# Sudaraka88/LDWeaver

Measured on AMD Instinct MI355X. Metric: MI SNP-pairs/sec, higher is better.
Workload: dtype i8

## Files before the change

### ldweaver_amd/csrc/ldw_apx.h

```cpp
#pragma once
#include "ldw_internal.h"
#include "ldw_epi.h"

namespace ldw {

constexpr int APX_TW = 128;
struct ApxGemmArgs {
    const uint64_t *panel_t, *panel_f;
    int RTpad, RFpad, M2;
    const uint8_t *dig_a, *dig_b;
    const int32_t *shift;
    int32_t *G;
    int lower_only;
    int fine;
    int fuse;
    const uint8_t *bin_t, *bin_f;
    const int2 *tab;
    int tab_nb;
    uint8_t *clean;
    const uint8_t *sr_mask;
    unsigned long long *skip_ctr;
    uint32_t *tile_list;
    unsigned int *n_live;
    int grid_wgs;
// ... 12 lines not shown
```

### ldweaver_amd/csrc/ldw_apx.hip

```cpp
#include <algorithm>
#include <cmath>
#include <cstdlib>

#include "ldw_apx.h"
#include "ldw_pairs.h"
#include "ldw_dev.h"

using namespace ldw;

namespace ldw {

namespace {
constexpr int64_t APX_PROD_CAP = 12000;
struct ProdTable {
    std::vector<int32_t> val;
    std::vector<uint8_t> a, b;
    ProdTable() {
        std::vector<std::pair<int32_t, std::pair<uint8_t, uint8_t>>> all;
        for (int x = 0; x <= 127; ++x)
            for (int y = x; y <= 127; ++y) all.push_back({x * y, {(uint8_t)x, (uint8_t)y}});
        std::sort(all.begin(), all.end());
        for (auto &e : all)
            if (val.empty() || val.back() != e.first) {
                val.push_back(e.first);
// ... 85 lines not shown
    c->apx.apx_ok = delta <= 4e-3 && Npad <= 30720 && M2 > 0;
    {
        char why[160];
        if (c->apx.apx_ok) snprintf(why, sizeof(why), c->apx.apx_fine ? "ok (block exponents per 32 positions)" : "ok");
        else if (!(delta <= 4e-3)) snprintf(why, sizeof(why), "delta %.3g > 4e-03 (dual-digit weights too coarse)", delta);
        else if (Npad > 30720) snprintf(why, sizeof(why), "Npad %lld > 30720 (digit arrays exceed the GEMM's LDS)", (long long)Npad);
        else snprintf(why, sizeof(why), "no macro step (Npad %lld)", (long long)Npad);
        c->apx.apx_gate = why;
    }
    return LDW_OK;
}

__global__ __launch_bounds__(256) void k_pack_panel(const uint64_t *__restrict__ Mbits, int64_t KW, const int32_t *__restrict__ rowlist,
                                                    int Rpad, int M2, uint64_t *__restrict__ panel, int interleave,
                                                    const int32_t *__restrict__ rowlist2 = nullptr, int Rpad2 = 0, uint64_t *__restrict__ panel2 = nullptr) {
    typedef unsigned long long u64x2 __attribute__((ext_vector_type(2)));
    typedef unsigned int u32x4 __attribute__((ext_vector_type(4)));
    if (blockIdx.y == 1) {
        rowlist = rowlist2;
        Rpad = Rpad2;
        panel = panel2;
    }
    const int r = blockIdx.x * 64 + (threadIdx.x & 63);
    if (r >= Rpad) return;
    const u64x2 *src = reinterpret_cast<const u64x2 *>(Mbits + (int64_t)rowlist[r] * KW);
    u32x4 *dst4 = reinterpret_cast<u32x4 *>(panel);
    for (int m = threadIdx.x >> 6; m < M2; m += 4) {
        u64x2 v = src[m];
        if (interleave) {
            const unsigned long long x = v[0], y = v[1];
            const unsigned long long ex = (x & 0xFFFFull) | ((x >> 16) & 0xFFFF0000ull) | ((y & 0xFFFFull) << 32) | ((y << 16) & 0xFFFF000000000000ull);
            const unsigned long long ox = ((x >> 16) & 0xFFFFull) | ((x >> 32) & 0xFFFF0000ull) | (((y >> 16) & 0xFFFFull) << 32) | (y & 0xFFFF000000000000ull);
            v[0] = ex;
            v[1] = ox;
        }
#pragma unroll
        for (int h = 0; h < 2; ++h) {
            const unsigned long long w = v[h];
            u32x4 o;
#pragma unroll
            for (int kk = 0; kk < 4; ++kk)
                o[kk] = (((unsigned int)(w >> (16 * kk)) & 0xFFu) << 3) | (((unsigned int)(w >> (16 * kk + 8)) & 0xFFu) << 19);
            dst4[((int64_t)m * Rpad + r) * 2 + h] = o;
        }
    }
}

int launch_pack_panel(ldw_ctx *c, const int32_t *rowlist, int Rpad, uint64_t *panel, hipStream_t st, const int32_t *rowlist2, int Rpad2, uint64_t *panel2) {
    const int rmax = (rowlist2 && Rpad2 > Rpad) ? Rpad2 : Rpad;
    hipLaunchKernelGGL(k_pack_panel, dim3((unsigned)((rmax + 63) / 64), rowlist2 ? 2u : 1u), dim3(256), 0, st, c->rows.Mbits.as<uint64_t>(), c->KW, rowlist, Rpad,
                       (int)(c->KW / 2), panel, c->apx.apx_fine ? 1 : 0, rowlist2, Rpad2, panel2);
    LDW_HIP(hipGetLastError());
    return LDW_OK;
}

typedef int v4i __attribute__((ext_vector_type(4)));
typedef int v16i __attribute__((ext_vector_type(16)));
constexpr int APX_MT = 4, APX_WPS = 2;

typedef unsigned int apx_u32x4 __attribute__((ext_vector_type(4)));
// ... 122 lines not shown
            S.bmin = v < S.bmin ? v : S.bmin;
            S.bmax = v > S.bmax ? v : S.bmax;
        }
        if (flags) {
            const uint4 f = *reinterpret_cast<const uint4 *>(flags + i);
            unsigned a = f.x & f.y & f.z & f.w, o = f.x | f.y | f.z | f.w;
            a &= a >> 16; a &= a >> 8;
            o |= o >> 16; o |= o >> 8;
            S.fand &= a & 0xFFu;
            S.forr |= o & 0xFFu;
        }
    }
    return S;
}

__global__ __launch_bounds__(256) void k_apx_live_tiles(ApxGemmArgs P) {
    constexpr int MT = APX_MT, NT = 2, TH = 32 * MT, TWd = 32 * NT;
    __shared__ unsigned int s_wave[4], s_base;
    const int ty = (int)blockIdx.x, ntx = P.RFpad / TWd;
    const int lane = threadIdx.x & 63, wave = threadIdx.x >> 6;
    const TileSummary T = apx_fold_rows(P.bin_t + (int64_t)ty * TH, P.rflag_t ? P.rflag_t + (int64_t)ty * TH : nullptr, TH);
    unsigned int n_pruned = 0;
    for (int tx0 = 0; tx0 < ntx; tx0 += 256) {
        const int tx = tx0 + (int)threadIdx.x;
        const bool valid = tx < ntx && !(P.lower_only && tx * TWd + TWd - 1 < ty * TH);
        bool pruned = false, all_binned = false;
        if (valid && !(P.sr_mask && P.sr_mask[(int64_t)((ty * TH) / 128) * (P.RFpad / 64) + tx] != 0)) {
            const TileSummary F = apx_fold_rows(P.bin_f + (int64_t)tx * TWd, P.rflag_f ? P.rflag_f + (int64_t)tx * TWd : nullptr, TWd);
            all_binned = T.bmax < P.tab_nb && F.bmax < P.tab_nb;
            if (P.rflag_t) {
                const unsigned kt = T.fand & PF_KIND, kf = F.fand & PF_KIND;
                pruned = kt >= 2u && kt == (T.forr & PF_KIND) && kf >= 2u && kf == (F.forr & PF_KIND) &&
                         ((T.fand & (kf == 2u ? PF_DEAD2 : PF_DEAD3)) != 0u || (F.fand & (kt == 2u ? PF_DEAD2 : PF_DEAD3)) != 0u);
            }
            if (!pruned && all_binned && (T.bmax - T.bmin + 1) * (F.bmax - F.bmin + 1) <= 64) {
                bool ok = true;
                for (int bt = T.bmin; bt <= T.bmax; ++bt)
                    for (int bf = F.bmin; bf <= F.bmax; ++bf) {
                        const int2 th = P.tab[bt * P.tab_nb + bf];
                        ok = ok && th.x < 0 && th.y == 2147483647;
                    }
                pruned = ok;
            }
        }
        if (pruned && all_binned) {
#pragma unroll
            for (int i = 0; i < MT; ++i)
#pragma unroll
                for (int h = 0; h < (NT * 32) / 64; ++h) P.clean[(int64_t)((ty * TH + 32 * i) / 32) * (P.RFpad / 64) + (tx * TWd) / 64 + h] = 1;
        }
        const bool live = valid && !pruned;
        const unsigned long long lm = __ballot(live);
        n_pruned += (unsigned int)__popcll(__ballot(valid && pruned));
        if (lane == 0) s_wave[wave] = (unsigned int)__popcll(lm);
        __syncthreads();
        if (threadIdx.x == 0) {
            const unsigned int tot = s_wave[0] + s_wave[1] + s_wave[2] + s_wave[3];
// ... 207 lines not shown
```

### ldweaver_amd/csrc/ldw_mi.hip

```cpp
#include <algorithm>
#include <chrono>
#include <cmath>
#include <cstring>
#include "ldw_prim.h"

#include "ldw_internal.h"
#include "ldw_dev.h"
#ifndef LDW_SCREEN_V
#define LDW_SCREEN_V 2
#endif
#ifndef LDW_SCREEN_WAVES
#define LDW_SCREEN_WAVES 6
#endif
#include "ldw_epi.h"
#include "ldw_pass_plan.h"
#include <future>

#include "ldw_apx.h"
#include "ldw_pairs.h"

using namespace ldw;

namespace ldw {
#include "ldw_mi_screen.inc"
// ... 73 lines not shown
        if (int rc = c->cand_val[s].reserve(cand * 8)) return rc;
        if (int rc = gx(c, s).reserve(RF * RF * 8)) return rc;
    }
    if (int rc = c->pair_sums.reserve((size_t)PAIR_PATHS * PAIR_SHARDS * cap * 16 * 8)) return rc;
    return LDW_OK;
}

int block_mi_dense(ldw_ctx *c, const int32_t *from_idx, int64_t nf, const int32_t *to_idx, int64_t nt, int quirk) {
    EmitArgs E;
    memset(&E, 0, sizeof(E));
    return run_block_mi(c, from_idx, nf, to_idx, nt, quirk, E);
}

void warm_mi() {
    hipFuncAttributes a;
    (void)hipFuncGetAttributes(&a, reinterpret_cast<const void *>(&k_zero4));
    (void)hipFuncGetAttributes(&a, reinterpret_cast<const void *>(&k_mi_screen<1, true>));
    (void)hipGetLastError();
}
}

extern "C" {

int ldw_mi_block(ldw_ctx *c, const int32_t *from_idx, int64_t nf, const int32_t *to_idx, int64_t nt, int quirk_mode,
                 double *MI_out, int on_device) {
    if (int rc = check_gpu(c)) return rc;
    LDW_REQUIRE(from_idx && to_idx && MI_out, LDW_ERR_ARG, "ldw_mi_block: null argument");
    LDW_REQUIRE(quirk_mode == LDW_QUIRK_REFERENCE || quirk_mode == LDW_QUIRK_INTENDED, LDW_ERR_ARG, "bad quirk mode");
    EmitArgs E;
    memset(&E, 0, sizeof(E));
    if (int rc = run_block_mi(c, from_idx, nf, to_idx, nt, quirk_mode, E)) return rc;
// ... 463 lines not shown
```

### ldweaver_amd/csrc/ldw_mi_block.inc

```

int upload_i32(ldw_ctx *c, ldw::DevBuf &buf, const std::vector<int32_t> &v) {
    if (int rc = buf.reserve(v.size() * 4 + 4)) return rc;
    if (!v.empty()) LDW_HIP(hipMemcpyAsync(buf.p, v.data(), v.size() * 4, hipMemcpyHostToDevice, c->stream));
    return LDW_OK;
}

struct SideLists {
    std::vector<int32_t> rowlist, lrow, pos;
    std::vector<uint8_t> cls;
    int Rpad = 0;
};

int build_side(ldw_ctx *c, const int32_t *idx, int64_t n, SideLists &S, const std::vector<int32_t> *order1 = nullptr) {
    S.lrow.assign((size_t)n, 0);
    S.rowlist.clear();
    S.pos.clear();
    S.cls.clear();
    const int32_t zero_row = (int32_t)c->rows.R;
    for (int64_t k = 0; k < n; ++k)
        LDW_REQUIRE(idx[k] >= 0 && idx[k] < c->L, LDW_ERR_ARG, "SNP index %d out of range 0..%lld", idx[k], (long long)c->L - 1);
    for (int cl : {1, 2, 4}) {
        const bool ordered = cl == 1 && order1 != nullptr;
        const int64_t cnt = ordered ? (int64_t)order1->size() : n;
        for (int64_t kk = 0; kk < cnt; ++kk) {
// ... 503 lines not shown
    }
    const bool maybe_on = getenv("LDW_NO_MAYBE") == nullptr;
    const bool use_maybe = maybe_on && !c->spec.maybe_off && fuse && use_pairs && c->knobs.screen == 1 && !E.lower_only && c->KW >= 32;
    unsigned int *maybe_n = nullptr;
    ApxMaybe *maybe_list = nullptr;
    MiniCol *mini_c = nullptr;
    MiniRow *mini_r = nullptr;
    if (use_maybe) {
        maybe_n = PL.hdr + PH_MAYBE_N;
        maybe_list = PL.maybe;
        if (int rc = place(M, c->apx_mini[s])) return rc;
        A.mini_c = mini_c = M.col;
        A.mini_r = mini_r = M.row;
    }
    if (phase == 1) {
        if (E.do_lr) {
            if (int rc = launch_pack_panel(c, D.rl_f, RFpad, c->panel[s][0].as<uint64_t>(), gs, lo_h->diag ? nullptr : D.rl_t, RTpad,
                                           lo_h->diag ? nullptr : c->panel[s][1].as<uint64_t>()))
                return rc;
        }
        {
            ZeroArgs Z;
            memset(&Z, 0, sizeof(Z));
            auto zero = [&Z](int k, const Carve::Range &r) {
                Z.p[k] = reinterpret_cast<uint4 *>(r.p);
                Z.n16[k] = r.n16();
            };
            zero(0, U.zeroed());
            if (use_pairs) zero(1, PL.zeroed());
            if (fuse) {
                Z.p[4] = reinterpret_cast<uint4 *>(c->apx_clean[s].p);
                Z.n16[4] = (unsigned int)(((size_t)(RTpad / 32) * (size_t)(RFpad / 64) + 15) / 16);
            }
            zero(5, B.zeroed());
            if (zero_hist) {
                Z.p[2] = reinterpret_cast<uint4 *>(zero_hist);
                Z.n16[2] = (unsigned int)((size_t)NBINS * 8 / 16 * (size_t)(lo_h->span ? lo_h->span : 1));
                Z.p[3] = reinterpret_cast<uint4 *>(zero_pick);
                Z.n16[3] = (unsigned int)(zero_pick_bytes / 16);
            }
            hipLaunchKernelGGL(k_zero4, dim3(16), dim3(256), 0, gs, Z);
        }
        const int nthr = std::max<int>(std::max<int>((int)nt, (int)g.nf_slots()), std::max<int>(RTpad, RFpad));
        hipLaunchKernelGGL(k_build_packs, dim3((unsigned)((nthr + 255) / 256), 2), dim3(256), 0, gs, A, D.perm, D.perm_t, (int)g.nf_slots(), 1, K.cp, K.cp_hi, K.rp,
                           K.rp_hi, K.rloc_f, K.rloc_t, B.bin_t, B.bin_f, RTpad, RFpad, sflag_f, sflag_t, rflag_f, rflag_t, mini_c, mini_r);
        LDW_HIP(hipGetLastError());
        ApxGemmArgs P;
        if (E.do_lr) {
            memset(&P, 0, sizeof(P));
            P.panel_f = c->panel[s][0].as<uint64_t>();
            P.panel_t = lo_h->diag ? P.panel_f : c->panel[s][1].as<uint64_t>();
            P.RTpad = RTpad;
            P.RFpad = RFpad;
            P.M2 = (int)(c->KW / 2);
            P.dig_a = c->apx.dig_a.as<uint8_t>();
            P.dig_b = c->apx.dig_b.as<uint8_t>();
            P.shift = c->apx.apx_shift.as<int32_t>();
            P.fine = c->apx.apx_fine ? 1 : 0;
            P.G = c->Gapx[s].as<int32_t>();
            P.lower_only = E.lower_only;
// ... 64 lines not shown
    if (need_exact && !band_early)
        if (int rc = launch_gemm_bits(c, c->rows.Mbits.as<uint64_t>(), c->KW, D.rl_t, RTpad, D.rl_f, RFpad, Gx.as<int64_t>(), c->wts.nlimbs, c->wts.digits.as<int8_t>(),
                                      E.lower_only, s2, 0, -1, band, band ? D.band_list : nullptr, D.n_band))
            return rc;
    if (use_pairs) {
        if (int rc = c->pair_sums.reserve((size_t)PAIR_PATHS * PAIR_SHARDS * A.pl_cap * 16 * 8)) return rc;
        if (int rc = launch_pairs_exact(c, A, ghist, c->pair_sums.as<int64_t>(), s2)) return rc;
    }
    if (need_exact) {
        EpiArgs Ax = A;
        Ax.G = Gx.as<int64_t>();
        Ax.E.apx = 0;
        Ax.pl_pairs = nullptr;
        launch_units(Ax, D, U, ghist, s2);
    }
    hipLaunchKernelGGL(k_apx_stats, dim3(1), dim3(64), 0, s2, U.counters, A.pl_n, A.pl_cap, A.E.scr_viol + 1);
    LDW_HIP(hipGetLastError());
    LDW_HIP(hipEventRecord(ev[2], s2));
    return LDW_OK;
}

void build_perm_tiles(ldw_ctx *c, const int32_t *from_idx, int64_t nf, std::vector<int32_t> &perm, const std::vector<int32_t> *order1 = nullptr) {
    perm.clear();
    for (int want : {1, 2, 3, 4, 0}) {
        if (want == 1 && order1) perm.insert(perm.end(), order1->begin(), order1->end());
        else
            for (int64_t k = 0; k < nf; ++k)
                if (c->rows.h_row0[from_idx[k] + 1] - c->rows.h_row0[from_idx[k]] == want) perm.push_back((int32_t)k);
        if (want != 3)
            while (perm.size() % 64) perm.push_back(-1);
    }
    if (perm.empty()) perm.assign(64, -1);
// ... 107 lines not shown
```

### ldweaver_amd/csrc/ldw_mi_eval.inc

```
#ifndef LDW_EPI_WAVES
#define LDW_EPI_WAVES 3
#endif
#ifndef LDW_EPI_FAST_WAVES
#define LDW_EPI_FAST_WAVES 5
#endif
#ifndef LDW_EPI_U11
#define LDW_EPI_U11 4
#endif
#ifndef LDW_EPI_U
#define LDW_EPI_U 2
#endif
struct EpiFastConst {
    double den, rY, hrcp, rxy0;
};
__device__ __forceinline__ bool col_is_fast_r(const ColMeta &M, uint32_t mb) { return col_is_fast(mb) && M.rb == (double)((int)(mb & 7) + 1); }

template <int MODE>
__device__ __forceinline__ void epi_fast_emit(const EmitArgs &E, const ColMeta &M, int a_loc, int b_loc, int sa, double mi, unsigned int *sh_hist) {
    if (E.write_dense) E.MI[(int64_t)a_loc + (int64_t)b_loc * E.nf] = mi;
    if (MODE == 0) return;
    if (a_loc == b_loc) return;
    const int seg = a_loc > b_loc ? 1 : 0;
    if (E.any_sr) {
        const ColInfo &c = M.ci;
// ... 328 lines not shown
                    g_viol_rec[k * 4 + 1] = (double)M.sb;
                    g_viol_rec[k * 4 + 2] = mi;
                    g_viol_rec[k * 4 + 3] = (double)A.E.spec_lo;
                }
            }
            continue;
        }
        emit_pair_spec(A.E, M.ci, a_loc, b_loc, R.sa, M.sb, mi, ghist);
    }
}

struct ZeroArgs {
    uint4 *p[6];
    unsigned int n16[6];
};
__global__ __launch_bounds__(256) void k_zero4(ZeroArgs Z) {
    const uint4 z = make_uint4(0u, 0u, 0u, 0u);
#pragma unroll
    for (int k = 0; k < 6; ++k)
        for (unsigned int i = blockIdx.x * 256u + threadIdx.x; i < Z.n16[k]; i += gridDim.x * 256u) Z.p[k][i] = z;
}

__global__ void k_apx_stats(const unsigned int *__restrict__ n_units, const unsigned int *__restrict__ pl_n, unsigned int pl_cap,
                            unsigned long long *__restrict__ acc) {
    if (threadIdx.x != 0 || blockIdx.x != 0) return;
    acc[0] += (unsigned long long)n_units[0] + n_units[1];
    unsigned long long k = 0;
    if (pl_n)
        for (int i = 0; i < PAIR_PATHS * PAIR_SHARDS; ++i) k += pl_n[i] > pl_cap ? pl_cap : pl_n[i];
    acc[1] += k;
    if (pl_n) acc[2] += (unsigned long long)pl_n[PH_MAYBE_N];
}

struct GenArgs {
    const double *MI;
    int nf, nt, lower_only, keep_sr, do_lr;
    const int32_t *idx_f, *idx_t, *POS;
    double g, sr_dist;
};

__device__ __forceinline__ bool gen_is_sr(const GenArgs &S, int a_loc, double pos1) {
    return circ_len(pos1, (double)S.POS[S.idx_f[a_loc]], S.g) <= S.sr_dist;
}

__global__ __launch_bounds__(256) void k_gen_count(GenArgs S, int32_t *__restrict__ cnt_u, int32_t *__restrict__ cnt_l,
                                                   unsigned long long *__restrict__ ghist) {
// ... 106 lines not shown
```

### ldweaver_amd/csrc/ldw_mi_items.inc

```

struct StageImage {
    struct Part {
        size_t off, bytes;
        const void *src;
        void (*point)(DevPtrs &, const char *);
    };
    Part part[18] = {};
    int n = 0;
    size_t bytes = 0;
    template <class T> static T elem_of(const T *DevPtrs::*);
    template <auto F> using Elem = decltype(elem_of(F));
    template <auto F> size_t array(const Elem<F> *src, size_t count) {
        part[n] = Part{bytes, count * sizeof(Elem<F>), src, [](DevPtrs &D, const char *p) { D.*F = reinterpret_cast<const Elem<F> *>(p); }};
        bytes = (bytes + part[n].bytes + 63) / 64 * 64;
        return part[n++].off;
    }
    void copy_to(char *image) const {
        for (int k = 0; k < n; ++k)
            if (part[k].src && part[k].bytes) memcpy(image + part[k].off, part[k].src, part[k].bytes);
    }
    void bind(DevPtrs &D, const char *image) const {
        for (int k = 0; k < n; ++k) part[k].point(D, image + part[k].off);
    }
};
// ... 425 lines not shown
    E.scr_mode = (hb.spec_B > 0 || !do_lr) && !E.write_dense && (!do_lr || speculation_pays(c, p)) ? c->knobs.screen : 0;
    const int64_t tot = hb.mixed ? c->wts.total_fixed_hi : c->wts.total_fixed;
    int bits = 0;
    while (bits < 62 && (tot >> bits) != 0) ++bits;
    E.scr_shift = bits > 31 ? bits - 31 : 0;
    E.scr_scale = (float)std::ldexp(1.0, E.scr_shift - c->wts.frac_bits + (hb.mixed ? 8 * LO_LIMBS : 0));
    E.scr_eps = SCREEN_EPS + (hb.mixed ? (float)lo_bound(c) : 0.0f);
    if (hb.apx) {
        apx_screen_params(c, E);
    }
    E.scr_viol = reinterpret_cast<unsigned long long *>(sl.lr_count + 1);
    hb.E = E;
    return LDW_OK;
}

int launch_pick(ldw_ctx *c, const HostBlock &hb, const ldw_mi_params *p, const SmallLayout &sl, hipStream_t st) {
    const int s = hb.slot;
    const unsigned int *pl_hdr = c->pairs[s].as<unsigned int>();
    if (hb.span) {
        PickSpanArgs S;
        memset(&S, 0, sizeof(S));
        for (int k = 0; k < hb.span; ++k) S.n_total[k] = (long long)hb.seg_lr_total[k];
        hipLaunchKernelGGL(k_pick_bucket_span, dim3((unsigned)hb.span), dim3(256), 0, st, c->hist[s].as<unsigned long long>(), p->lr_retain_links,
                           p->lr_links_approx, hb.spec_B, S, reinterpret_cast<char *>(sl.pick[s]), PICK_STRIDE,
                           pl_hdr, pair_cap_for(hb.nf, hb.nt, hb.span));
        LDW_HIP(hipGetLastError());
        return LDW_OK;
    }
    if (!p->sr_only) {
        const bool pl = hb.apx && c->knobs.screen == 1;
        hipLaunchKernelGGL(k_pick_bucket, dim3(1), dim3(256), 0, st, c->hist[s].as<unsigned long long>(), p->lr_retain_links,
                           p->lr_links_approx, hb.spec_B, (long long)hb.n_lr_total, sl.pick[s],
                           pl ? pl_hdr : nullptr, pair_cap_for(hb.nf, hb.nt));
        LDW_HIP(hipGetLastError());
    }
    return LDW_OK;
}

static void fill_dev_ptrs(ldw_ctx *c, HostBlock &hb) {
    hb.img.bind(hb.D, c->dstage[hb.pin_slot >= 0 ? hb.pin_slot : hb.slot].as<char>() + hb.stage_base);
}

int submit_upload(ldw_ctx *c, HostBlock &hb) {
    if (hb.uploaded) return LDW_OK;
    const int s = hb.slot;
    const int stg = hb.pin_slot >= 0 ? hb.pin_slot : s;
    if (int rc = c->dstage[stg].reserve(hb.total)) return rc;
    if (c->done_recorded[s]) LDW_HIP(hipStreamWaitEvent(c->copy_stream, c->ev_done[s], 0));
// ... 337 lines not shown
    bool missed = false;
    if (do_lr && hb.spec_B >= 0 && hp->n > 0 && !hp->spec_ok) {
        EmitArgs E = hb.E;
        E.write_dense = 1;
        E.spec_B = -1;
        E.keep_sr = 0;
        E.scr_mode = 0;
        hb.spec_B = -1;
        LDW_HIP(hipMemsetAsync(c->hist[s].p, 0, (size_t)NBINS * 8, c->stream));
        LDW_HIP(hipMemsetAsync(sl.pick[s], 0, sizeof(ldw::PickOut), c->stream));
        hipEvent_t dummy[6] = {c->ev[3], c->ev[3], c->ev[4], c->ev[3], c->ev[5], c->ev[3]};
        E.apx = 0;
        if (int rc = launch_block_mi(c, hb.D, hb.nf, hb.nt, hb.RFpad, hb.RTpad, p->quirk_mode, E, dummy, (hb.mixed || hb.apx) ? 3 : 2,
                                     &gx(c, s), nullptr, c->hist[s].as<unsigned long long>()))
            return rc;
        if (int rc = launch_pick(c, hb, p, sl, c->stream)) return rc;
        if (int rc = launch_gather(c, hb, E, sl)) return rc;
        LDW_HIP(hipMemcpyAsync(c->pin_pick[s], sl.pick[s], sizeof(ldw::PickOut), hipMemcpyDeviceToHost, c->stream));
        LDW_HIP(hipStreamSynchronize(c->stream));
        ++c->cnt.spec_misses;
        note_overflow(c, hp->over);
        missed = true;
    }
    note_block(c, hb, 0, hp, do_lr, missed || hb.force_plain);
    if (int rc = read_lr_count(c)) return rc;
    if (int rc = select_rows(c, sel_in(c, hb, sl, 0, do_lr ? (int64_t)hp->n_cand : 0), do_lr, sl)) return rc;
    return end_item(c, hb, sl);
}

int run_block_alone(ldw_ctx *c, const HostBlock &span, int k, const ldw_mi_params *p, const SmallLayout &sl, bool force_plain) {
    HostBlock hb;
// ... 181 lines not shown
```

### ldweaver_amd/csrc/ldw_mi_screen.inc

```

static inline ldw::DevBuf &gx(ldw_ctx *c, int s) { return s == 0 ? c->G : (s == 1 ? c->G2 : c->G3); }

__global__ __launch_bounds__(256) void k_build_packs(EpiArgs A, const int32_t *__restrict__ perm_f, const int32_t *__restrict__ perm_t,
                                                     int nf_slots, int with_hi, ColMeta *__restrict__ cp, ColMeta *__restrict__ cp_hi,
                                                     RowPack *__restrict__ rp, RowPack *__restrict__ rp_hi, float *__restrict__ rloc_f,
                                                     float *__restrict__ rloc_t, uint8_t *__restrict__ bin_t = nullptr,
                                                     uint8_t *__restrict__ bin_f = nullptr, int RTpad = 0, int RFpad = 0,
                                                     uint8_t *__restrict__ sflag_f = nullptr, uint8_t *__restrict__ sflag_t = nullptr,
                                                     uint8_t *__restrict__ rflag_f = nullptr, uint8_t *__restrict__ rflag_t = nullptr,
                                                     MiniCol *__restrict__ mini_c = nullptr, MiniRow *__restrict__ mini_r = nullptr) {
    const int i = blockIdx.x * 256 + threadIdx.x;
    const bool square = A.nf == A.nt;
    const double lvl = A.E.spec_lo - (double)A.E.scr_eps;
    auto prune_flags = [&](int snp, uint32_t meta, double r) -> unsigned {
        const int n = (int)(meta & 7);
        const uint32_t full = (2u << n) - 1u;
        if (!(n == 1 || n == 2) || ((meta >> 3) & full) != full || r != (double)(n + 1)) return 0u;
        const double *sp = A.snp_sup + (int64_t)snp * 4 + (A.quirk == LDW_QUIRK_REFERENCE ? 2 : 0);
        return (unsigned)(n + 1) | (sp[0] < lvl ? PF_DEAD2 : 0u) | (sp[1] < lvl ? PF_DEAD3 : 0u);
    };
    int my_bt = 255, my_bf = 255;
    const bool to_side = blockIdx.y == 0;
    if (!to_side && i < A.nf) rloc_f[i] = (float)A.r[A.idx_f[i]];
    if (to_side && i < A.nt) rloc_t[i] = (float)A.r[A.idx_t[i]];
    if (to_side && i < A.nt) {
        ColMeta m;
        load_col(A, perm_t, square, i, m, false);
        if (A.span) {
            m.bl -= m.ci.pad[1];
            m.rq = A.r[A.idx_f[m.bl]];
        }
        cp[i] = m;
        if ((m.mb & 7) == 1 && col_is_fast(m.mb) && m.rb == 2.0) my_bt = m.pad2 & 63;
        if (sflag_t) {
            const unsigned f = prune_flags(m.sb, m.mb, m.rb);
            sflag_t[i] = (uint8_t)f;
            for (int j = 0; j < (int)(m.mb & 7); ++j) rflag_t[m.rb0 + j] = (uint8_t)f;
// ... 16 lines not shown
        if (sflag_f) {
            const unsigned f = ok ? prune_flags(P.R.sa, P.R.ma, P.R.ra) : PF_PAD;
            sflag_f[i] = (uint8_t)f;
            if (ok)
                for (int j = 0; j < P.R.na; ++j) rflag_f[P.R.ra0 + j] = (uint8_t)f;
        }
        if (with_hi) {
#pragma unroll
            for (int k = 0; k < 5; ++k) P.R.pa[k] = A.lo.slot_pfix_hi[(int64_t)P.R.sa * 5 + k];
            rp_hi[i] = P;
            if (mini_r) mini_r[i] = MiniRow{(int32_t)P.R.pa[0], (int32_t)P.R.pa[1], P.R.pXf[0], P.R.pXf[1], (float)P.R.ra, (float)P.R.rta, P.a_loc, P.R.sa};
        }
    }
    if (to_side && bin_t && i < RTpad) bin_t[i] = (uint8_t)my_bt;
    if (!to_side && bin_f && i < RFpad) bin_f[i] = (uint8_t)my_bf;
}

struct PendPairs {
    unsigned int m[2];
    int q_base;
};
__device__ __forceinline__ void mark_pair(PendPairs &pp, int which, bool mine, int q) {
    if (mine) pp.m[which] |= 1u << (q - pp.q_base);
}
__device__ __forceinline__ void flush_pairs(const EpiArgs &A, int path, unsigned int mask, int q_base, int tile, int sa, const ColMeta *cmw) {
    const int lane = threadIdx.x & 63;
    const unsigned int cnt = (unsigned int)__popc(mask);
    if (__ballot(cnt != 0u) == 0ull) return;
    unsigned int incl = cnt;
#pragma unroll
// ... 691 lines not shown
```

### ldweaver_amd/csrc/ldw_mi_select.inc

```
struct PickOut {
    long long n;
    long long lo, hi;
    long long n_below;
    double index, prob;
    int B;
    int spec_ok;
    int B_true, over;
    unsigned long long n_cand;
    long long n_kept;
    double disc_thresh;
    long long kstart;
    long long n_below_true;
};

__device__ __forceinline__ void pick_bucket_body(const unsigned long long *__restrict__ hist, double lr_retain, double lr_approx, int spec_B,
                                                 long long n_total, PickOut *__restrict__ out, const unsigned int *__restrict__ pl_n,
                                                 unsigned int pl_cap) {
    __shared__ long long part[256];
    __shared__ long long s_lo;
    constexpr int PER = NBINS / 256;
    const int t = threadIdx.x;
    long long loc[PER], sum = 0;
#pragma unroll
    for (int k = 0; k < PER; ++k) {
// ... 58 lines not shown
                    for (int i = 0; i < PAIR_PATHS * PAIR_SHARDS; ++i) over |= pl_n[i] > pl_cap ? 1 : 0;
                    over |= pl_n[PH_MAYBE_OVER] > pl_cap ? 2 : 0;
                }
                out->over = over;
                out->spec_ok = over ? 0 : 1;
            }
            cum += loc[k];
        }
    } else if (t == 0) {
        out->n_cand = 0;
    }
}

__global__ __launch_bounds__(256) void k_pick_bucket(const unsigned long long *__restrict__ hist, double lr_retain,
                                                     double lr_approx, int spec_B, long long n_total,
                                                     PickOut *__restrict__ out, const unsigned int *__restrict__ pl_n, unsigned int pl_cap) {
    pick_bucket_body(hist, lr_retain, lr_approx, spec_B, n_total, out, pl_n, pl_cap);
}

struct PickSpanArgs {
    long long n_total[LDW_SPAN_MAX];
};
__global__ __launch_bounds__(256) void k_pick_bucket_span(const unsigned long long *__restrict__ hist, double lr_retain, double lr_approx, int spec_B,
                                                          PickSpanArgs S, char *__restrict__ picks, size_t pick_stride,
                                                          const unsigned int *__restrict__ pl_n, unsigned int pl_cap) {
    const int k = (int)blockIdx.x;
    pick_bucket_body(hist + (size_t)k * NBINS, lr_retain, lr_approx, spec_B, S.n_total[k], reinterpret_cast<PickOut *>(picks + (size_t)k * pick_stride), pl_n,
                     pl_cap);
}

struct GatherArgs {
    const double *MI;
    const ColInfo *cols;
    int nf, nt, lower_only;
};

__global__ __launch_bounds__(256) void k_lr_gather(GatherArgs S, PickOut *__restrict__ pick, uint64_t *__restrict__ ckey,
                                                   uint64_t *__restrict__ cval) {
    const int B = pick->B;
    if (B >= NBINS) return;
    const double lo_val = B > 0 ? bucket_lo(B) : 0.0;
    const int b0 = blockIdx.x * 16;
    for (int bb = 0; bb < 16; ++bb) {
// ... 561 lines not shown
```

### ldweaver_amd/csrc/ldw_slots.h

```cpp
#pragma once
#include "ldw_carve.h"

namespace ldw {

struct ColInfo {
    int32_t s[3], e[3];
    int32_t pad[2];
    int64_t off_u, off_l;
};

struct ColMeta {
    int32_t sb;
    uint32_t mb;
    int32_t rb0, bl;
    double rb;
    double rq;
    double pYd[5];
    int64_t pb[5];
    float pYf[5];
    int32_t pad2;
#ifdef LDW_COLMETA_PAD
    char padx[LDW_COLMETA_PAD];
#endif
    ColInfo ci;
// ... 94 lines not shown
        : hdr(take<unsigned int>(PH_WORDS)), lists(take<PairEnt>((int64_t)PAIR_PATHS * PAIR_SHARDS * pl_cap)), maybe(take<ApxMaybe>(maybe_cap)) {}
    Range zeroed() const { return cover(hdr); }
};

struct BinsLayout : Carve {
    Slot<uint8_t> bin_t, bin_f;
    Slot<uint8_t> rflag_t, rflag_f;
    Slot<unsigned int> n_live;
    Slot<uint8_t> sflag_t, sflag_f;
    Slot<uint32_t> tile_list;
    explicit BinsLayout(const SlotGeom &g)
        : bin_t(take<uint8_t>(g.RTpad)), bin_f(take<uint8_t>(g.RFpad)), rflag_t(take<uint8_t>(g.RTpad)), rflag_f(take<uint8_t>(g.RFpad)),
          n_live(take<unsigned int>(1)), sflag_t(take<uint8_t>(g.nt)), sflag_f(take<uint8_t>(g.nf_slots())),
          tile_list(take<uint32_t>((g.RTpad / 64) * (g.RFpad / 64))) {}
    Range zeroed() const { return cover(rflag_t, rflag_f, n_live); }
};

struct MiniLayout : Carve {
    Slot<MiniCol> col;
    Slot<MiniRow> row;
    explicit MiniLayout(const SlotGeom &g) : col(take<MiniCol>(g.nt)), row(take<MiniRow>(g.nf_slots())) {}
};

constexpr uint64_t PAIR_CAP = 1u << 18;
inline uint32_t pair_cap_of(int64_t nf, int64_t nt, int nseg) {
    const uint64_t top = nseg > 4 ? 2 * PAIR_CAP : PAIR_CAP;
    uint64_t want = (uint64_t)nf * (uint64_t)nt / PAIR_SHARDS + 1, cap = 1u << 12;
    while (cap < want && cap < top) cap <<= 1;
    return (uint32_t)cap;
}
// ... 17 lines not shown
```

Baseline: 179.5 billion.

## Fuse zeroing, pack building and panel packing into one prep kernel

Merges the zero kernel, the build-packs kernel and the panel-pack kernel into a single k_apx_prep launch that partitions its workgroups by role. It also folds the stats update into the pick kernel when the low-rank path runs, and precomputes per-bin threshold bitmasks in LDS so the live-tile pruning check becomes a bitmask OR instead of a table loop. The fused launch relies on rflag clearing happening inside build_packs_side rather than in a separate zero pass, which changes the ordering assumptions between zeroing and writing. It also assumes tab_nb is at most 64 and that tab holds at least 64x64 entries.

```diff
diff --git a/ldweaver_amd/csrc/ldw_apx.h b/ldweaver_amd/csrc/ldw_apx.h
--- a/ldweaver_amd/csrc/ldw_apx.h
+++ b/ldweaver_amd/csrc/ldw_apx.h
@@ -1,6 +1,7 @@
 #pragma once
 #include "ldw_internal.h"
 #include "ldw_epi.h"
+#include "ldw_apx_panel.h"
 
 namespace ldw {
 
diff --git a/ldweaver_amd/csrc/ldw_apx.hip b/ldweaver_amd/csrc/ldw_apx.hip
--- a/ldweaver_amd/csrc/ldw_apx.hip
+++ b/ldweaver_amd/csrc/ldw_apx.hip
@@ -123,36 +123,8 @@
 __global__ __launch_bounds__(256) void k_pack_panel(const uint64_t *__restrict__ Mbits, int64_t KW, const int32_t *__restrict__ rowlist,
                                                     int Rpad, int M2, uint64_t *__restrict__ panel, int interleave,
                                                     const int32_t *__restrict__ rowlist2 = nullptr, int Rpad2 = 0, uint64_t *__restrict__ panel2 = nullptr) {
-    typedef unsigned long long u64x2 __attribute__((ext_vector_type(2)));
-    typedef unsigned int u32x4 __attribute__((ext_vector_type(4)));
-    if (blockIdx.y == 1) {
-        rowlist = rowlist2;
-        Rpad = Rpad2;
-        panel = panel2;
-    }
-    const int r = blockIdx.x * 64 + (threadIdx.x & 63);
-    if (r >= Rpad) return;
-    const u64x2 *src = reinterpret_cast<const u64x2 *>(Mbits + (int64_t)rowlist[r] * KW);
-    u32x4 *dst4 = reinterpret_cast<u32x4 *>(panel);
-    for (int m = threadIdx.x >> 6; m < M2; m += 4) {
-        u64x2 v = src[m];
-        if (interleave) {
-            const unsigned long long x = v[0], y = v[1];
-            const unsigned long long ex = (x & 0xFFFFull) | ((x >> 16) & 0xFFFF0000ull) | ((y & 0xFFFFull) << 32) | ((y << 16) & 0xFFFF000000000000ull);
-            const unsigned long long ox = ((x >> 16) & 0xFFFFull) | ((x >> 32) & 0xFFFF0000ull) | (((y >> 16) & 0xFFFFull) << 32) | (y & 0xFFFF000000000000ull);
-            v[0] = ex;
-            v[1] = ox;
-        }
-#pragma unroll
-        for (int h = 0; h < 2; ++h) {
-            const unsigned long long w = v[h];
-            u32x4 o;
-#pragma unroll
-            for (int kk = 0; kk < 4; ++kk)
-                o[kk] = (((unsigned int)(w >> (16 * kk)) & 0xFFu) << 3) | (((unsigned int)(w >> (16 * kk + 8)) & 0xFFu) << 19);
-            dst4[((int64_t)m * Rpad + r) * 2 + h] = o;
-        }
-    }
+    if (blockIdx.y == 1) apx_pack_panel_wg(blockIdx.x, Mbits, KW, rowlist2, Rpad2, M2, panel2, interleave);
+    else apx_pack_panel_wg(blockIdx.x, Mbits, KW, rowlist, Rpad, M2, panel, interleave);
 }
 
 int launch_pack_panel(ldw_ctx *c, const int32_t *rowlist, int Rpad, uint64_t *panel, hipStream_t st, const int32_t *rowlist2, int Rpad2, uint64_t *panel2) {
@@ -305,12 +277,37 @@
     return S;
 }
 
+__device__ __forceinline__ TileSummary apx_fold_group128(const uint8_t *__restrict__ bins, const uint8_t *__restrict__ flags) {
+    const int l8 = threadIdx.x & 7;
+    TileSummary S = apx_fold_rows(bins + 16 * l8, flags ? flags + 16 * l8 : nullptr, 16);
+#pragma unroll
+    for (int o = 1; o < 8; o <<= 1) {
+        const int mn = __shfl_xor(S.bmin, o), mx = __shfl_xor(S.bmax, o);
+        const unsigned fa = (unsigned)__shfl_xor((int)S.fand, o), fo = (unsigned)__shfl_xor((int)S.forr, o);
+        S.bmin = mn < S.bmin ? mn : S.bmin;
+        S.bmax = mx > S.bmax ? mx : S.bmax;
+        S.fand &= fa;
+        S.forr |= fo;
+    }
+    return S;
+}
+
 __global__ __launch_bounds__(256) void k_apx_live_tiles(ApxGemmArgs P) {
     constexpr int MT = APX_MT, NT = 2, TH = 32 * MT, TWd = 32 * NT;
+    static_assert(TH == 128 && TWd == 64, "the folds are written for groups of 128 to-rows and 64 from-rows");
     __shared__ unsigned int s_wave[4], s_base;
+    __shared__ unsigned long long s_cond[64];
     const int ty = (int)blockIdx.x, ntx = P.RFpad / TWd;
     const int lane = threadIdx.x & 63, wave = threadIdx.x >> 6;
-    const TileSummary T = apx_fold_rows(P.bin_t + (int64_t)ty * TH, P.rflag_t ? P.rflag_t + (int64_t)ty * TH : nullptr, TH);
+#pragma unroll
+    for (int k = 0; k < 16; ++k) {
+        const int bt = wave + 4 * k;
+        const int2 th = P.tab[bt * 64 + lane];
+        const unsigned long long m = __ballot(!(th.x < 0 && th.y == 2147483647));
+        if (lane == 0) s_cond[bt] = m;
+    }
+    const TileSummary T = apx_fold_group128(P.bin_t + (int64_t)ty * TH, P.rflag_t ? P.rflag_t + (int64_t)ty * TH : nullptr);
+    __syncthreads();
     unsigned int n_pruned = 0;
     for (int tx0 = 0; tx0 < ntx; tx0 += 256) {
         const int tx = tx0 + (int)threadIdx.x;
@@ -325,13 +322,11 @@
                          ((T.fand & (kf == 2u ? PF_DEAD2 : PF_DEAD3)) != 0u || (F.fand & (kt == 2u ? PF_DEAD2 : PF_DEAD3)) != 0u);
             }
             if (!pruned && all_binned && (T.bmax - T.bmin + 1) * (F.bmax - F.bmin + 1) <= 64) {
-                bool ok = true;
-                for (int bt = T.bmin; bt <= T.bmax; ++bt)
-                    for (int bf = F.bmin; bf <= F.bmax; ++bf) {
-                        const int2 th = P.tab[bt * P.tab_nb + bf];
-                        ok = ok && th.x < 0 && th.y == 2147483647;
-                    }
-                pruned = ok;
+                const int wf = F.bmax - F.bmin + 1;
+                const unsigned long long cols = (wf >= 64 ? ~0ull : ((1ull << wf) - 1ull)) << F.bmin;
+                unsigned long long cond = 0ull;
+                for (int bt = T.bmin; bt <= T.bmax; ++bt) cond |= s_cond[bt] & cols;
+                pruned = cond == 0ull;
             }
         }
         if (pruned && all_binned) {
diff --git a/ldweaver_amd/csrc/ldw_apx_panel.h b/ldweaver_amd/csrc/ldw_apx_panel.h
--- /dev/null
+++ b/ldweaver_amd/csrc/ldw_apx_panel.h
@@ -0,0 +1,36 @@
+#pragma once
+#include <hip/hip_runtime.h>
+#include <cstdint>
+
+namespace ldw {
+
+__device__ __forceinline__ void apx_pack_panel_wg(unsigned wg, const uint64_t *__restrict__ Mbits, int64_t KW, const int32_t *__restrict__ rowlist, int Rpad,
+                                                  int M2, uint64_t *__restrict__ panel, int interleave) {
+    typedef unsigned long long u64x2 __attribute__((ext_vector_type(2)));
+    typedef unsigned int u32x4 __attribute__((ext_vector_type(4)));
+    const int r = (int)wg * 64 + (threadIdx.x & 63);
+    if (r >= Rpad) return;
+    const u64x2 *src = reinterpret_cast<const u64x2 *>(Mbits + (int64_t)rowlist[r] * KW);
+    u32x4 *dst4 = reinterpret_cast<u32x4 *>(panel);
+    for (int m = threadIdx.x >> 6; m < M2; m += 4) {
+        u64x2 v = src[m];
+        if (interleave) {
+            const unsigned long long x = v[0], y = v[1];
+            const unsigned long long ex = (x & 0xFFFFull) | ((x >> 16) & 0xFFFF0000ull) | ((y & 0xFFFFull) << 32) | ((y << 16) & 0xFFFF000000000000ull);
+            const unsigned long long ox = ((x >> 16) & 0xFFFFull) | ((x >> 32) & 0xFFFF0000ull) | (((y >> 16) & 0xFFFFull) << 32) | (y & 0xFFFF000000000000ull);
+            v[0] = ex;
+            v[1] = ox;
+        }
+#pragma unroll
+        for (int h = 0; h < 2; ++h) {
+            const unsigned long long w = v[h];
+            u32x4 o;
+#pragma unroll
+            for (int kk = 0; kk < 4; ++kk)
+                o[kk] = (((unsigned int)(w >> (16 * kk)) & 0xFFu) << 3) | (((unsigned int)(w >> (16 * kk + 8)) & 0xFFu) << 19);
+            dst4[((int64_t)m * Rpad + r) * 2 + h] = o;
+        }
+    }
+}
+
+}
diff --git a/ldweaver_amd/csrc/ldw_mi.hip b/ldweaver_amd/csrc/ldw_mi.hip
--- a/ldweaver_amd/csrc/ldw_mi.hip
+++ b/ldweaver_amd/csrc/ldw_mi.hip
@@ -111,7 +111,7 @@
 
 void warm_mi() {
     hipFuncAttributes a;
-    (void)hipFuncGetAttributes(&a, reinterpret_cast<const void *>(&k_zero4));
+    (void)hipFuncGetAttributes(&a, reinterpret_cast<const void *>(&k_apx_prep));
     (void)hipFuncGetAttributes(&a, reinterpret_cast<const void *>(&k_mi_screen<1, true>));
     (void)hipGetLastError();
 }
diff --git a/ldweaver_amd/csrc/ldw_mi_block.inc b/ldweaver_amd/csrc/ldw_mi_block.inc
--- a/ldweaver_amd/csrc/ldw_mi_block.inc
+++ b/ldweaver_amd/csrc/ldw_mi_block.inc
@@ -541,36 +541,46 @@
         A.mini_r = mini_r = M.row;
     }
     if (phase == 1) {
+        ZeroArgs Z;
+        memset(&Z, 0, sizeof(Z));
+        auto zero = [&Z](int k, const Carve::Range &r) {
+            Z.p[k] = reinterpret_cast<uint4 *>(r.p);
+            Z.n16[k] = r.n16();
+        };
+        zero(0, U.zeroed());
+        if (use_pairs) zero(1, PL.zeroed());
+        if (fuse) {
+            Z.p[4] = reinterpret_cast<uint4 *>(c->apx_clean[s].p);
+            Z.n16[4] = (unsigned int)(((size_t)(RTpad / 32) * (size_t)(RFpad / 64) + 15) / 16);
+        }
+        zero(5, B.zeroed_by_prep());
+        if (zero_hist) {
+            Z.p[2] = reinterpret_cast<uint4 *>(zero_hist);
+            Z.n16[2] = (unsigned int)((size_t)NBINS * 8 / 16 * (size_t)(lo_h->span ? lo_h->span : 1));
+            Z.p[3] = reinterpret_cast<uint4 *>(zero_pick);
+            Z.n16[3] = (unsigned int)(zero_pick_bytes / 16);
+        }
+        const PackOut O{K.cp, K.cp_hi, K.rp, K.rp_hi, K.rloc_f, K.rloc_t, B.bin_t, B.bin_f, RTpad, RFpad, sflag_f, sflag_t, rflag_f, rflag_t, mini_c, mini_r,
+                        D.rl_t, D.rl_f, (int32_t)c->rows.R};
+        PanelArgs Pn;
+        memset(&Pn, 0, sizeof(Pn));
         if (E.do_lr) {
-            if (int rc = launch_pack_panel(c, D.rl_f, RFpad, c->panel[s][0].as<uint64_t>(), gs, lo_h->diag ? nullptr : D.rl_t, RTpad,
-                                           lo_h->diag ? nullptr : c->panel[s][1].as<uint64_t>()))
-                return rc;
-        }
-        {
-            ZeroArgs Z;
-            memset(&Z, 0, sizeof(Z));
-            auto zero = [&Z](int k, const Carve::Range &r) {
-                Z.p[k] = reinterpret_cast<uint4 *>(r.p);
-                Z.n16[k] = r.n16();
-            };
-            zero(0, U.zeroed());
-            if (use_pairs) zero(1, PL.zeroed());
-            if (fuse) {
-                Z.p[4] = reinterpret_cast<uint4 *>(c->apx_clean[s].p);
-                Z.n16[4] = (unsigned int)(((size_t)(RTpad / 32) * (size_t)(RFpad / 64) + 15) / 16);
+            Pn.Mbits = c->rows.Mbits.as<uint64_t>();
+            Pn.KW = c->KW;
+            Pn.M2 = (int)(c->KW / 2);
+            Pn.interleave = c->apx.apx_fine ? 1 : 0;
+            Pn.rowlist[0] = D.rl_f;
+            Pn.Rpad[0] = RFpad;
+            Pn.panel[0] = c->panel[s][0].as<uint64_t>();
+            if (!lo_h->diag) {
+                Pn.rowlist[1] = D.rl_t;
+                Pn.Rpad[1] = RTpad;
+                Pn.panel[1] = c->panel[s][1].as<uint64_t>();
             }
-            zero(5, B.zeroed());
-            if (zero_hist) {
-                Z.p[2] = reinterpret_cast<uint4 *>(zero_hist);
-                Z.n16[2] = (unsigned int)((size_t)NBINS * 8 / 16 * (size_t)(lo_h->span ? lo_h->span : 1));
-                Z.p[3] = reinterpret_cast<uint4 *>(zero_pick);
-                Z.n16[3] = (unsigned int)(zero_pick_bytes / 16);
-            }
-            hipLaunchKernelGGL(k_zero4, dim3(16), dim3(256), 0, gs, Z);
         }
         const int nthr = std::max<int>(std::max<int>((int)nt, (int)g.nf_slots()), std::max<int>(RTpad, RFpad));
-        hipLaunchKernelGGL(k_build_packs, dim3((unsigned)((nthr + 255) / 256), 2), dim3(256), 0, gs, A, D.perm, D.perm_t, (int)g.nf_slots(), 1, K.cp, K.cp_hi, K.rp,
-                           K.rp_hi, K.rloc_f, K.rloc_t, B.bin_t, B.bin_f, RTpad, RFpad, sflag_f, sflag_t, rflag_f, rflag_t, mini_c, mini_r);
+        const PrepGrid Gd(nthr, true, Pn.Rpad[0], Pn.Rpad[1]);
+        hipLaunchKernelGGL(k_apx_prep, dim3(Gd.total()), dim3(256), 0, gs, Gd, A, D.perm, D.perm_t, (int)g.nf_slots(), O, Z, Pn);
         LDW_HIP(hipGetLastError());
         ApxGemmArgs P;
         if (E.do_lr) {
@@ -665,8 +675,10 @@
         Ax.pl_pairs = nullptr;
         launch_units(Ax, D, U, ghist, s2);
     }
-    hipLaunchKernelGGL(k_apx_stats, dim3(1), dim3(64), 0, s2, U.counters, A.pl_n, A.pl_cap, A.E.scr_viol + 1);
-    LDW_HIP(hipGetLastError());
+    if (!E.do_lr) {
+        hipLaunchKernelGGL(k_apx_stats, dim3(1), dim3(64), 0, s2, U.counters, A.pl_n, A.pl_cap, A.E.scr_viol + 1);
+        LDW_HIP(hipGetLastError());
+    }
     LDW_HIP(hipEventRecord(ev[2], s2));
     return LDW_OK;
 }
diff --git a/ldweaver_amd/csrc/ldw_mi_eval.inc b/ldweaver_amd/csrc/ldw_mi_eval.inc
--- a/ldweaver_amd/csrc/ldw_mi_eval.inc
+++ b/ldweaver_amd/csrc/ldw_mi_eval.inc
@@ -366,22 +366,46 @@
     uint4 *p[6];
     unsigned int n16[6];
 };
-__global__ __launch_bounds__(256) void k_zero4(ZeroArgs Z) {
+__device__ __forceinline__ void zero_ranges_wg(const ZeroArgs &Z, unsigned int wg, unsigned int nwg) {
     const uint4 z = make_uint4(0u, 0u, 0u, 0u);
 #pragma unroll
     for (int k = 0; k < 6; ++k)
-        for (unsigned int i = blockIdx.x * 256u + threadIdx.x; i < Z.n16[k]; i += gridDim.x * 256u) Z.p[k][i] = z;
-}
-
-__global__ void k_apx_stats(const unsigned int *__restrict__ n_units, const unsigned int *__restrict__ pl_n, unsigned int pl_cap,
-                            unsigned long long *__restrict__ acc) {
-    if (threadIdx.x != 0 || blockIdx.x != 0) return;
+        for (unsigned int i = wg * 256u + threadIdx.x; i < Z.n16[k]; i += nwg * 256u) Z.p[k][i] = z;
+}
+
+struct PanelArgs {
+    const uint64_t *Mbits;
+    int64_t KW;
+    const int32_t *rowlist[2];
+    int Rpad[2];
+    uint64_t *panel[2];
+    int M2, interleave;
+};
+__global__ __launch_bounds__(256) void k_apx_prep(PrepGrid Gd, EpiArgs A, const int32_t *__restrict__ perm_f, const int32_t *__restrict__ perm_t, int nf_slots,
+                                                  PackOut O, ZeroArgs Z, PanelArgs Pn) {
+    unsigned int wg;
+    const int part = Gd.part_of(blockIdx.x, wg);
+    if (part == PrepGrid::PACKS_T || part == PrepGrid::PACKS_F) build_packs_side(A, perm_f, perm_t, nf_slots, 1, O, part == PrepGrid::PACKS_T, (int)(wg * 256u + threadIdx.x));
+    else if (part == PrepGrid::ZERO) zero_ranges_wg(Z, wg, Gd.first[PrepGrid::ZERO + 1] - Gd.first[PrepGrid::ZERO]);
+    else {
+        const int k = part == PrepGrid::PANEL_T ? 1 : 0;
+        apx_pack_panel_wg(wg, Pn.Mbits, Pn.KW, Pn.rowlist[k], Pn.Rpad[k], Pn.M2, Pn.panel[k], Pn.interleave);
+    }
+}
+
+__device__ __forceinline__ void apx_stats_body(const unsigned int *__restrict__ n_units, const unsigned int *__restrict__ pl_n, unsigned int pl_cap,
+                                               unsigned long long *__restrict__ acc) {
     acc[0] += (unsigned long long)n_units[0] + n_units[1];
     unsigned long long k = 0;
     if (pl_n)
         for (int i = 0; i < PAIR_PATHS * PAIR_SHARDS; ++i) k += pl_n[i] > pl_cap ? pl_cap : pl_n[i];
     acc[1] += k;
     if (pl_n) acc[2] += (unsigned long long)pl_n[PH_MAYBE_N];
+}
+__global__ void k_apx_stats(const unsigned int *__restrict__ n_units, const unsigned int *__restrict__ pl_n, unsigned int pl_cap,
+                            unsigned long long *__restrict__ acc) {
+    if (threadIdx.x != 0 || blockIdx.x != 0) return;
+    apx_stats_body(n_units, pl_n, pl_cap, acc);
 }
 
 struct GenArgs {
diff --git a/ldweaver_amd/csrc/ldw_mi_items.inc b/ldweaver_amd/csrc/ldw_mi_items.inc
--- a/ldweaver_amd/csrc/ldw_mi_items.inc
+++ b/ldweaver_amd/csrc/ldw_mi_items.inc
@@ -463,16 +463,19 @@
     return LDW_OK;
 }
 
-int launch_pick(ldw_ctx *c, const HostBlock &hb, const ldw_mi_params *p, const SmallLayout &sl, hipStream_t st) {
+int launch_pick(ldw_ctx *c, const HostBlock &hb, const ldw_mi_params *p, const SmallLayout &sl, hipStream_t st, bool with_stats = true) {
     const int s = hb.slot;
     const unsigned int *pl_hdr = c->pairs[s].as<unsigned int>();
+    const bool stats = hb.apx && with_stats;
+    const unsigned int *st_units = stats ? c->apx_units[s].as<unsigned int>() : nullptr;
+    unsigned long long *st_acc = stats ? hb.E.scr_viol + 1 : nullptr;
     if (hb.span) {
         PickSpanArgs S;
         memset(&S, 0, sizeof(S));
         for (int k = 0; k < hb.span; ++k) S.n_total[k] = (long long)hb.seg_lr_total[k];
         hipLaunchKernelGGL(k_pick_bucket_span, dim3((unsigned)hb.span), dim3(256), 0, st, c->hist[s].as<unsigned long long>(), p->lr_retain_links,
                            p->lr_links_approx, hb.spec_B, S, reinterpret_cast<char *>(sl.pick[s]), PICK_STRIDE,
-                           pl_hdr, pair_cap_for(hb.nf, hb.nt, hb.span));
+                           pl_hdr, pair_cap_for(hb.nf, hb.nt, hb.span), st_units, st_acc);
         LDW_HIP(hipGetLastError());
         return LDW_OK;
     }
@@ -480,7 +483,7 @@
         const bool pl = hb.apx && c->knobs.screen == 1;
         hipLaunchKernelGGL(k_pick_bucket, dim3(1), dim3(256), 0, st, c->hist[s].as<unsigned long long>(), p->lr_retain_links,
                            p->lr_links_approx, hb.spec_B, (long long)hb.n_lr_total, sl.pick[s],
-                           pl ? pl_hdr : nullptr, pair_cap_for(hb.nf, hb.nt));
+                           pl ? pl_hdr : nullptr, pair_cap_for(hb.nf, hb.nt), st_units, st_acc);
         LDW_HIP(hipGetLastError());
     }
     return LDW_OK;
@@ -848,7 +851,7 @@
         if (int rc = launch_block_mi(c, hb.D, hb.nf, hb.nt, hb.RFpad, hb.RTpad, p->quirk_mode, E, dummy, (hb.mixed || hb.apx) ? 3 : 2,
                                      &gx(c, s), nullptr, c->hist[s].as<unsigned long long>()))
             return rc;
-        if (int rc = launch_pick(c, hb, p, sl, c->stream)) return rc;
+        if (int rc = launch_pick(c, hb, p, sl, c->stream, false)) return rc;
         if (int rc = launch_gather(c, hb, E, sl)) return rc;
         LDW_HIP(hipMemcpyAsync(c->pin_pick[s], sl.pick[s], sizeof(ldw::PickOut), hipMemcpyDeviceToHost, c->stream));
         LDW_HIP(hipStreamSynchronize(c->stream));
diff --git a/ldweaver_amd/csrc/ldw_mi_screen.inc b/ldweaver_amd/csrc/ldw_mi_screen.inc
--- a/ldweaver_amd/csrc/ldw_mi_screen.inc
+++ b/ldweaver_amd/csrc/ldw_mi_screen.inc
@@ -1,15 +1,28 @@
 
 static inline ldw::DevBuf &gx(ldw_ctx *c, int s) { return s == 0 ? c->G : (s == 1 ? c->G2 : c->G3); }
 
-__global__ __launch_bounds__(256) void k_build_packs(EpiArgs A, const int32_t *__restrict__ perm_f, const int32_t *__restrict__ perm_t,
-                                                     int nf_slots, int with_hi, ColMeta *__restrict__ cp, ColMeta *__restrict__ cp_hi,
-                                                     RowPack *__restrict__ rp, RowPack *__restrict__ rp_hi, float *__restrict__ rloc_f,
-                                                     float *__restrict__ rloc_t, uint8_t *__restrict__ bin_t = nullptr,
-                                                     uint8_t *__restrict__ bin_f = nullptr, int RTpad = 0, int RFpad = 0,
-                                                     uint8_t *__restrict__ sflag_f = nullptr, uint8_t *__restrict__ sflag_t = nullptr,
-                                                     uint8_t *__restrict__ rflag_f = nullptr, uint8_t *__restrict__ rflag_t = nullptr,
-                                                     MiniCol *__restrict__ mini_c = nullptr, MiniRow *__restrict__ mini_r = nullptr) {
-    const int i = blockIdx.x * 256 + threadIdx.x;
+struct PackOut {
+    ColMeta *cp, *cp_hi;
+    RowPack *rp, *rp_hi;
+    float *rloc_f, *rloc_t;
+    uint8_t *bin_t, *bin_f;
+    int RTpad, RFpad;
+    uint8_t *sflag_f, *sflag_t, *rflag_f, *rflag_t;
+    MiniCol *mini_c;
+    MiniRow *mini_r;
+    const int32_t *rl_t, *rl_f;
+    int32_t zero_row;
+};
+__device__ __forceinline__ void build_packs_side(const EpiArgs &A, const int32_t *__restrict__ perm_f, const int32_t *__restrict__ perm_t, int nf_slots,
+                                                 int with_hi, const PackOut &O, bool to_side, int i) {
+    ColMeta *__restrict__ cp = O.cp, *__restrict__ cp_hi = O.cp_hi;
+    RowPack *__restrict__ rp = O.rp, *__restrict__ rp_hi = O.rp_hi;
+    float *__restrict__ rloc_f = O.rloc_f, *__restrict__ rloc_t = O.rloc_t;
+    uint8_t *__restrict__ bin_t = O.bin_t, *__restrict__ bin_f = O.bin_f;
+    const int RTpad = O.RTpad, RFpad = O.RFpad;
+    uint8_t *__restrict__ sflag_f = O.sflag_f, *__restrict__ sflag_t = O.sflag_t, *__restrict__ rflag_f = O.rflag_f, *__restrict__ rflag_t = O.rflag_t;
+    MiniCol *__restrict__ mini_c = O.mini_c;
+    MiniRow *__restrict__ mini_r = O.mini_r;
     const bool square = A.nf == A.nt;
     const double lvl = A.E.spec_lo - (double)A.E.scr_eps;
     auto prune_flags = [&](int snp, uint32_t meta, double r) -> unsigned {
@@ -20,7 +33,6 @@
         return (unsigned)(n + 1) | (sp[0] < lvl ? PF_DEAD2 : 0u) | (sp[1] < lvl ? PF_DEAD3 : 0u);
     };
     int my_bt = 255, my_bf = 255;
-    const bool to_side = blockIdx.y == 0;
     if (!to_side && i < A.nf) rloc_f[i] = (float)A.r[A.idx_f[i]];
     if (to_side && i < A.nt) rloc_t[i] = (float)A.r[A.idx_t[i]];
     if (to_side && i < A.nt) {
@@ -67,6 +79,20 @@
     }
     if (to_side && bin_t && i < RTpad) bin_t[i] = (uint8_t)my_bt;
     if (!to_side && bin_f && i < RFpad) bin_f[i] = (uint8_t)my_bf;
+    if (to_side && rflag_t && O.rl_t && i < RTpad && O.rl_t[i] >= O.zero_row) rflag_t[i] = 0;
+    if (!to_side && rflag_f && O.rl_f && i < RFpad && O.rl_f[i] >= O.zero_row) rflag_f[i] = 0;
+}
+
+__global__ __launch_bounds__(256) void k_build_packs(EpiArgs A, const int32_t *__restrict__ perm_f, const int32_t *__restrict__ perm_t,
+                                                     int nf_slots, int with_hi, ColMeta *__restrict__ cp, ColMeta *__restrict__ cp_hi,
+                                                     RowPack *__restrict__ rp, RowPack *__restrict__ rp_hi, float *__restrict__ rloc_f,
+                                                     float *__restrict__ rloc_t, uint8_t *__restrict__ bin_t = nullptr,
+                                                     uint8_t *__restrict__ bin_f = nullptr, int RTpad = 0, int RFpad = 0,
+                                                     uint8_t *__restrict__ sflag_f = nullptr, uint8_t *__restrict__ sflag_t = nullptr,
+                                                     uint8_t *__restrict__ rflag_f = nullptr, uint8_t *__restrict__ rflag_t = nullptr,
+                                                     MiniCol *__restrict__ mini_c = nullptr, MiniRow *__restrict__ mini_r = nullptr) {
+    const PackOut O{cp, cp_hi, rp, rp_hi, rloc_f, rloc_t, bin_t, bin_f, RTpad, RFpad, sflag_f, sflag_t, rflag_f, rflag_t, mini_c, mini_r, nullptr, nullptr, 0};
+    build_packs_side(A, perm_f, perm_t, nf_slots, with_hi, O, blockIdx.y == 0, (int)(blockIdx.x * 256 + threadIdx.x));
 }
 
 struct PendPairs {
diff --git a/ldweaver_amd/csrc/ldw_mi_select.inc b/ldweaver_amd/csrc/ldw_mi_select.inc
--- a/ldweaver_amd/csrc/ldw_mi_select.inc
+++ b/ldweaver_amd/csrc/ldw_mi_select.inc
@@ -96,8 +96,10 @@
 
 __global__ __launch_bounds__(256) void k_pick_bucket(const unsigned long long *__restrict__ hist, double lr_retain,
                                                      double lr_approx, int spec_B, long long n_total,
-                                                     PickOut *__restrict__ out, const unsigned int *__restrict__ pl_n, unsigned int pl_cap) {
+                                                     PickOut *__restrict__ out, const unsigned int *__restrict__ pl_n, unsigned int pl_cap,
+                                                     const unsigned int *__restrict__ st_units = nullptr, unsigned long long *__restrict__ st_acc = nullptr) {
     pick_bucket_body(hist, lr_retain, lr_approx, spec_B, n_total, out, pl_n, pl_cap);
+    if (st_acc && threadIdx.x == 0) apx_stats_body(st_units, pl_n, pl_cap, st_acc);
 }
 
 struct PickSpanArgs {
@@ -105,10 +107,12 @@
 };
 __global__ __launch_bounds__(256) void k_pick_bucket_span(const unsigned long long *__restrict__ hist, double lr_retain, double lr_approx, int spec_B,
                                                           PickSpanArgs S, char *__restrict__ picks, size_t pick_stride,
-                                                          const unsigned int *__restrict__ pl_n, unsigned int pl_cap) {
+                                                          const unsigned int *__restrict__ pl_n, unsigned int pl_cap,
+                                                          const unsigned int *__restrict__ st_units = nullptr, unsigned long long *__restrict__ st_acc = nullptr) {
     const int k = (int)blockIdx.x;
     pick_bucket_body(hist + (size_t)k * NBINS, lr_retain, lr_approx, spec_B, S.n_total[k], reinterpret_cast<PickOut *>(picks + (size_t)k * pick_stride), pl_n,
                      pl_cap);
+    if (st_acc && k == 0 && threadIdx.x == 0) apx_stats_body(st_units, pl_n, pl_cap, st_acc);
 }
 
 struct GatherArgs {
diff --git a/ldweaver_amd/csrc/ldw_slots.h b/ldweaver_amd/csrc/ldw_slots.h
--- a/ldweaver_amd/csrc/ldw_slots.h
+++ b/ldweaver_amd/csrc/ldw_slots.h
@@ -132,6 +132,30 @@
           n_live(take<unsigned int>(1)), sflag_t(take<uint8_t>(g.nt)), sflag_f(take<uint8_t>(g.nf_slots())),
           tile_list(take<uint32_t>((g.RTpad / 64) * (g.RFpad / 64))) {}
     Range zeroed() const { return cover(rflag_t, rflag_f, n_live); }
+    Range zeroed_by_prep() const { return cover(n_live); }
+};
+
+struct PrepGrid {
+    enum Part : int { PACKS_T = 0, PACKS_F, ZERO, PANEL_F, PANEL_T, PARTS };
+    static constexpr unsigned ZERO_WGS = 16;
+    unsigned first[PARTS + 1];
+    static unsigned wgs(int64_t items, int per_wg) { return items > 0 ? (unsigned)((items + per_wg - 1) / per_wg) : 0u; }
+    PrepGrid(int64_t pack_items, bool zero, int64_t panel_rows_f, int64_t panel_rows_t) {
+        const unsigned n[PARTS] = {wgs(pack_items, 256), wgs(pack_items, 256), zero ? ZERO_WGS : 0u, wgs(panel_rows_f, 64), wgs(panel_rows_t, 64)};
+        first[0] = 0;
+        for (int k = 0; k < PARTS; ++k) first[k + 1] = first[k] + n[k];
+    }
+    unsigned total() const { return first[PARTS]; }
+    unsigned count(int part) const { return first[part + 1] - first[part]; }
+#if defined(__HIPCC__)
+    __host__ __device__
+#endif
+    int part_of(unsigned wg, unsigned &local) const {
+        int k = 0;
+        while (k + 1 < PARTS && wg >= first[k + 1]) ++k;
+        local = wg - first[k];
+        return k;
+    }
 };
 
 struct MiniLayout : Carve {
```

Measured after the change: 179.0 billion. Within noise of the previous version (-0.2%).
